# CrashCartCapital/rust-local-rag

Hardware: AMD Instinct MI355X
Metric: queries/sec, 768-d cosine top-100 over 10M chunks (single query, f32) (higher is better)
Workload: dtype f32

## Files before the change

rust-local-rag_amd/csrc/q8.hip:

```cpp
#include "common.h"
#include "kernels.h"
#include "../../include/rlr_gpu.h"

#include <algorithm>
#include <cstdlib>

namespace rlr {

namespace {

typedef unsigned int u32x4 __attribute__((ext_vector_type(4)));

__device__ inline float wave_max_abs(float v)
{
#pragma unroll
    for (int off = 32; off > 0; off >>= 1)
        v = fmaxf(v, __shfl_xor(v, off));
    return v;
}

__device__ inline float wave_add_all(float v)
{
#pragma unroll
    for (int off = 32; off > 0; off >>= 1)
        v += __shfl_xor(v, off);
    return v;
}

template <bool F16>
__global__ __launch_bounds__(256) void q8_build_kernel(const void *__restrict__ rows, uint32_t pitch_bytes, uint32_t dim,
                                                       uint32_t row_begin, uint32_t n_rows, uint8_t *__restrict__ q8,
                                                       float *__restrict__ scale, uint32_t *__restrict__ stats)
{
    const int lane = threadIdx.x & 63;
    const uint32_t row = row_begin + blockIdx.x * 4 + (threadIdx.x >> 6);
    if (row >= n_rows)
        return;
    const unsigned char *rowp = static_cast<const unsigned char *>(rows) + static_cast<size_t>(row) * pitch_bytes;
    auto elem = [&](uint32_t e) -> float {
        if constexpr (F16)
            return h2f(reinterpret_cast<const uint16_t *>(rowp)[e]);
        else
            return reinterpret_cast<const float *>(rowp)[e];
    };
    float m = 0.0f;
    bool has_nan = false, has_inf = false;
    for (uint32_t e = lane; e < dim; e += 64) {
        const float v = elem(e);
        has_nan |= v != v;
        has_inf |= __builtin_fabsf(v) > 3.4028234e38f;
        m = fmaxf(m, __builtin_fabsf(v));
    }
    has_nan = __ballot(has_nan) != 0;
    has_inf = __ballot(has_inf) != 0;
    const bool bad = has_nan || has_inf;
    m = wave_max_abs(m);
    const float s = (bad || m == 0.0f) ? 1.0f : m / 127.0f;
    float err2 = 0.0f;
    uint8_t *out = q8 + static_cast<size_t>(row) * dim;
    for (uint32_t e = lane; e < dim; e += 64) {
        const float v = bad ? 0.0f : elem(e);
        float k = __builtin_rintf(v / s);
        k = fminf(fmaxf(k, -127.0f), 127.0f);
        const float d = v - s * k;
        err2 += d * d;
        out[e] = static_cast<uint8_t>(static_cast<int>(k) + 128);
    }
    err2 = wave_add_all(err2);
    if (lane == 0) {
        scale[row] = bad ? __builtin_bit_cast(float, 0x7FC00000u) : s;
        if (has_inf && !has_nan)
            atomicOr(&stats[2], 1u);
        const float delta = __builtin_sqrtf(err2) * 1.001f + 1e-30f;
        if (!bad) {
            atomicMax(&stats[0], __builtin_bit_cast(uint32_t, delta));
            atomicMax(&stats[1], __builtin_bit_cast(uint32_t, s));
        }
    }
}

template <int B>
__device__ inline float ubyte_f32(uint32_t w)
{
    return static_cast<float>((w >> (8 * B)) & 0xFFu);
}

__device__ inline float dot16_u8(u32x4 x, const float (&q)[16], float acc)
{
    acc = __builtin_fmaf(ubyte_f32<0>(x[0]), q[0], acc);
    acc = __builtin_fmaf(ubyte_f32<1>(x[0]), q[1], acc);
    acc = __builtin_fmaf(ubyte_f32<2>(x[0]), q[2], acc);
    acc = __builtin_fmaf(ubyte_f32<3>(x[0]), q[3], acc);
    acc = __builtin_fmaf(ubyte_f32<0>(x[1]), q[4], acc);
    acc = __builtin_fmaf(ubyte_f32<1>(x[1]), q[5], acc);
    acc = __builtin_fmaf(ubyte_f32<2>(x[1]), q[6], acc);
    acc = __builtin_fmaf(ubyte_f32<3>(x[1]), q[7], acc);
    acc = __builtin_fmaf(ubyte_f32<0>(x[2]), q[8], acc);
    acc = __builtin_fmaf(ubyte_f32<1>(x[2]), q[9], acc);
    acc = __builtin_fmaf(ubyte_f32<2>(x[2]), q[10], acc);
    acc = __builtin_fmaf(ubyte_f32<3>(x[2]), q[11], acc);
    acc = __builtin_fmaf(ubyte_f32<0>(x[3]), q[12], acc);
    acc = __builtin_fmaf(ubyte_f32<1>(x[3]), q[13], acc);
    acc = __builtin_fmaf(ubyte_f32<2>(x[3]), q[14], acc);
    acc = __builtin_fmaf(ubyte_f32<3>(x[3]), q[15], acc);
    return acc;
}

template <int R, int L>
__global__ __launch_bounds__(256) void q8_scan_kernel(const uint8_t *__restrict__ q8, const float *__restrict__ scale,
                                                      const float *__restrict__ query, float *__restrict__ scores,
                                                      uint32_t *__restrict__ g_hist, uint32_t n_rows, uint32_t dim,
                                                      uint32_t group_rows)
{
    __shared__ uint32_t s_hist[kHistBins];
    const int tid = threadIdx.x;
    const int lane = tid & 63;
    const int wave = __builtin_amdgcn_readfirstlane(tid >> 6);
    for (int i = tid; i < kHistBins; i += 256)
        s_hist[i] = 0;
    const uint32_t p16 = dim / 16;
    bool active[L];
    float qv[L][16];
    float qs = 0.0f;
#pragma unroll
    for (int l = 0; l < L; ++l) {
        active[l] = static_cast<uint32_t>(lane + 64 * l) < p16;
#pragma unroll
        for (int b = 0; b < 16; ++b) {
            qv[l][b] = active[l] ? query[(lane + 64 * l) * 16 + b] : 0.0f;
            qs += qv[l][b];
        }
    }
    const float bias = 128.0f * qs;
    __syncthreads();

    const uint32_t n_groups = (n_rows + group_rows - 1) / group_rows;
    const uint32_t n_waves = gridDim.x * 4;
    for (uint32_t g = blockIdx.x * 4 + wave; g < n_groups; g += n_waves) {
        const uint32_t row0 = g * group_rows;
        const uint32_t nr = min(group_rows, n_rows - row0);
        float mine = 0.0f;
        for (uint32_t r = 0; r < nr; r += R) {
            u32x4 x[R][L];
            float sc[R];
#pragma unroll
            for (int rr = 0; rr < R; ++rr) {
                const uint32_t row = min(row0 + r + rr, row0 + nr - 1);
                const u32x4 *p = reinterpret_cast<const u32x4 *>(q8 + static_cast<size_t>(row) * dim) + lane;
#pragma unroll
                for (int l = 0; l < L; ++l)
                    x[rr][l] = active[l] ? __builtin_nontemporal_load(p + 64 * l)
                                         : u32x4{0x80808080u, 0x80808080u, 0x80808080u, 0x80808080u};
                sc[rr] = scale[row];
            }
#pragma unroll
            for (int rr = 0; rr < R; ++rr) {
                float acc = -bias;
#pragma unroll
                for (int l = 0; l < L; ++l)
                    acc = dot16_u8(x[rr][l], qv[l], acc);
                const float tot = wave_sum(acc);
                const float v = sc[rr] * tot;
                if (static_cast<uint32_t>(lane) == r + rr)
                    mine = v;
            }
        }
        if (static_cast<uint32_t>(lane) < nr) {
            scores[row0 + lane] = mine;
            if (g_hist)
                atomicAdd(&s_hist[score_key(mine) >> 21], 1u);
        }
    }
    if (g_hist) {
        __syncthreads();
        for (int i = tid; i < kHistBins; i += 256) {
            const uint32_t c = s_hist[i];
            if (c)
                atomicAdd(&g_hist[i], c);
        }
    }
}

template <int G, int NL, int NB>
__global__ __launch_bounds__(256) void q8_scan_packed_kernel(const uint8_t *__restrict__ q8, const float *__restrict__ scale,
                                                             const float *__restrict__ query, float *__restrict__ scores,
                                                             uint32_t *__restrict__ g_hist, uint32_t n_rows, uint32_t dim,
                                                             uint32_t group_rows)
{
    constexpr int RI = G * NB;
    static_assert(RI <= 64, "a group parks one score per lane");
    __shared__ uint32_t s_hist[kHistBins];
    const int tid = threadIdx.x;
    const int lane = tid & 63;
    const int wave = __builtin_amdgcn_readfirstlane(tid >> 6);
    for (int i = tid; i < kHistBins; i += 256)
        s_hist[i] = 0;
    const uint32_t p16 = dim / 16;
    uint32_t rib[NL], off[NL];
    float qv[NL][16], nbias[NL];
#pragma unroll
    for (int j = 0; j < NL; ++j) {
        const uint32_t u = static_cast<uint32_t>(j * 64 + lane);
        rib[j] = u / p16;
        const uint32_t seg = u - rib[j] * p16;
        off[j] = seg * 16;
        float qs = 0.0f;
#pragma unroll
        for (int b = 0; b < 16; ++b) {
            qv[j][b] = query[seg * 16 + b];
            qs += qv[j][b];
        }
        nbias[j] = -128.0f * qs;
    }
    __syncthreads();

    const uint32_t n_groups = (n_rows + group_rows - 1) / group_rows;
    const uint32_t n_waves = gridDim.x * 4;
    for (uint32_t g = blockIdx.x * 4 + wave; g < n_groups; g += n_waves) {
        const uint32_t row0 = g * group_rows;
        const uint32_t nr = min(group_rows, n_rows - row0);
        const uint32_t last = row0 + nr - 1;
        const float my_scale = scale[min(row0 + static_cast<uint32_t>(lane), last)];
        float mine = 0.0f;
        for (uint32_t r = 0; r < nr; r += RI) {
            u32x4 x[NB][NL];
#pragma unroll
            for (int bb = 0; bb < NB; ++bb)
#pragma unroll
                for (int j = 0; j < NL; ++j) {
                    const uint32_t row = min(row0 + r + bb * G + rib[j], last);
                    x[bb][j] = __builtin_nontemporal_load(reinterpret_cast<const u32x4 *>(q8 + static_cast<size_t>(row) * dim + off[j]));
                }
#pragma unroll
            for (int bb = 0; bb < NB; ++bb) {
                float acc[NL];
#pragma unroll
                for (int j = 0; j < NL; ++j)
                    acc[j] = dot16_u8(x[bb][j], qv[j], nbias[j]);
#pragma unroll
                for (int rb = 0; rb < G; ++rb) {
                    float part = 0.0f;
#pragma unroll
                    for (int j = 0; j < NL; ++j)
                        part += rib[j] == static_cast<uint32_t>(rb) ? acc[j] : 0.0f;
                    const float tot = wave_sum(part);
                    if (static_cast<uint32_t>(lane) == r + bb * G + rb)
                        mine = tot;
                }
            }
        }
        if (static_cast<uint32_t>(lane) < nr) {
            const float v = my_scale * mine;
            scores[row0 + lane] = v;
            if (g_hist)
                atomicAdd(&s_hist[score_key(v) >> 21], 1u);
        }
    }
    if (g_hist) {
        __syncthreads();
        for (int i = tid; i < kHistBins; i += 256) {
            const uint32_t c = s_hist[i];
            if (c)
                atomicAdd(&g_hist[i], c);
        }
    }
}

}

hipError_t launch_q8_build(const void *rows, uint32_t pitch16, uint32_t dim, int dtype, uint32_t row_begin, uint32_t n_rows,
                           void *q8, float *scale, uint32_t *stats, hipStream_t s)
{
    if (row_begin >= n_rows)
        return hipSuccess;
    const uint32_t blocks = (n_rows - row_begin + 3) / 4;
    if (dtype == RLR_F16)
        hipLaunchKernelGGL(q8_build_kernel<true>, dim3(blocks), dim3(256), 0, s, rows, pitch16 * 16, dim, row_begin, n_rows,
                           static_cast<uint8_t *>(q8), scale, stats);
    else
        hipLaunchKernelGGL(q8_build_kernel<false>, dim3(blocks), dim3(256), 0, s, rows, pitch16 * 16, dim, row_begin, n_rows,
                           static_cast<uint8_t *>(q8), scale, stats);
    return hipGetLastError();
}

hipError_t launch_q8_scan(const void *q8, const float *scale, uint32_t n_rows, uint32_t dim, const float *query,
                          float *scores, uint32_t *hist, int n_cu, hipStream_t s)
{
    if (n_rows == 0)
        return hipSuccess;
    static const int tune = [] {
        const char *v = getenv("RLR_Q8_VARIANT");
        return v ? static_cast<int>(strtol(v, nullptr, 0)) : 0;
    }();
    const int r = (tune & 0xFF) ? (tune & 0xFF) : 8;
    const uint32_t bpc = ((tune >> 8) & 0xFF) ? ((tune >> 8) & 0xFF) : 8;
    uint32_t group = ((tune >> 16) & 0xFF) ? ((tune >> 16) & 0xFF) : 32;
    group = std::max<uint32_t>(static_cast<uint32_t>(r), group / r * r);
    const uint32_t n_groups = (n_rows + group - 1) / group;
    const uint32_t blocks = std::max<uint32_t>(1, std::min<uint32_t>((n_groups + 3) / 4, static_cast<uint32_t>(n_cu) * bpc));
    const uint8_t *p = static_cast<const uint8_t *>(q8);
    static const bool packed = [] {
        const char *v = getenv("RLR_Q8_PACKED");
        return !(v && v[0] == '0');
    }();
    if (packed) {
        const uint32_t p16 = dim / 16;
#define RLR_Q8_PACKED_CASE(G_, NL_, NB_, GROUP_, BPC_)                                                                \
    if (p16 * G_ == NL_ * 64) {                                                                                      \
        const uint32_t pg = GROUP_;                                                                                  \
        const uint32_t pgroups = (n_rows + pg - 1) / pg;                                                             \
        const uint32_t pbpc = ((tune >> 8) & 0xFF) ? ((tune >> 8) & 0xFF) : BPC_;                                    \
        const uint32_t pblocks = std::max<uint32_t>(1, std::min<uint32_t>((pgroups + 3) / 4, static_cast<uint32_t>(n_cu) * pbpc)); \
        hipLaunchKernelGGL((q8_scan_packed_kernel<G_, NL_, NB_>), dim3(pblocks), dim3(256), 0, s, p, scale, query, scores, \
                           hist, n_rows, dim, pg);                                                                   \
        return hipGetLastError();                                                                                    \
    }
        RLR_Q8_PACKED_CASE(4, 3, 2, 32, 2)
        RLR_Q8_PACKED_CASE(8, 3, 1, 32, 4)
        RLR_Q8_PACKED_CASE(2, 3, 4, 32, 4)
        RLR_Q8_PACKED_CASE(2, 1, 8, 32, 8)
        RLR_Q8_PACKED_CASE(4, 1, 8, 32, 8)
        RLR_Q8_PACKED_CASE(8, 1, 8, 64, 8)
#undef RLR_Q8_PACKED_CASE
    }
    if (dim > 1024) {
        hipLaunchKernelGGL((q8_scan_kernel<4, 2>), dim3(blocks), dim3(256), 0, s, p, scale, query, scores, hist, n_rows, dim, group);
        return hipGetLastError();
    }
    switch (r) {
    case 4: hipLaunchKernelGGL((q8_scan_kernel<4, 1>), dim3(blocks), dim3(256), 0, s, p, scale, query, scores, hist, n_rows, dim, group); break;
    case 16: hipLaunchKernelGGL((q8_scan_kernel<16, 1>), dim3(blocks), dim3(256), 0, s, p, scale, query, scores, hist, n_rows, dim, group); break;
    default: hipLaunchKernelGGL((q8_scan_kernel<8, 1>), dim3(blocks), dim3(256), 0, s, p, scale, query, scores, hist, n_rows, dim, group); break;
    }
    return hipGetLastError();
}

float q8_arith_eps(uint32_t dim, float scale_max, float q_norm)
{
    return 32.0f * 5.9604645e-8f * 256.0f * __builtin_sqrtf(static_cast<float>(dim)) * q_norm * scale_max * 1.0625f;
}

}
```

Before: 224.5.

## Score int8 chunks with sdot4 against a three-plane integer query

Quantises the query into a 24-bit fixed-point integer split into three signed int8 planes. Each u8 chunk row is then scored with sdot4 integer dot products instead of per-byte float conversion plus FMA, and the three partial sums are recombined in double. Cross-lane reductions become integer DPP/shuffle fold trees that sum several rows at once rather than doing a full wave reduction per row. The default packed config for dim 768 changes to 4 rows per batch with one block per CU. This trades float ALU work for int dot instructions but adds query preprocessing, a fallback path for non-finite queries, and a small change in rounding behaviour.

```diff
diff --git a/rust-local-rag_amd/csrc/q8.hip b/rust-local-rag_amd/csrc/q8.hip
--- a/rust-local-rag_amd/csrc/q8.hip
+++ b/rust-local-rag_amd/csrc/q8.hip
@@ -79,6 +79,103 @@
     }
 }
 
+
+constexpr int kQ8Unit = 127 * 65793;
+
+__device__ inline bool q8_query_max(const float *__restrict__ query, uint32_t dim, int lane, float *qmax)
+{
+    float m = 0.0f;
+    bool bad = false;
+    for (uint32_t e = lane; e < dim; e += 64) {
+        const float a = __builtin_fabsf(query[e]);
+        bad |= !(a <= 3.4028234e38f);
+        m = fmaxf(m, a);
+    }
+    m = wave_max_abs(m);
+    *qmax = m;
+    return __ballot(bad) == 0 && m != 0.0f;
+}
+
+__device__ inline void q8_planes(const float *__restrict__ q16, bool active, double inv, u32x4 (&pl)[3])
+{
+#pragma unroll
+    for (int p = 0; p < 3; ++p)
+        pl[p] = u32x4{0u, 0u, 0u, 0u};
+#pragma unroll
+    for (int b = 0; b < 16; ++b) {
+        const double v = active ? static_cast<double>(q16[b]) : 0.0;
+        const int q = static_cast<int>(__builtin_rint(v * inv));
+        const int d0 = static_cast<int>(static_cast<int8_t>(q & 0xFF));
+        const int q1 = (q - d0) >> 8;
+        const int d1 = static_cast<int>(static_cast<int8_t>(q1 & 0xFF));
+        const int d2 = (q1 - d1) >> 8;
+        const int sh = 8 * (b & 3);
+        pl[0][b >> 2] |= static_cast<uint32_t>(d0 & 0xFF) << sh;
+        pl[1][b >> 2] |= static_cast<uint32_t>(d1 & 0xFF) << sh;
+        pl[2][b >> 2] |= static_cast<uint32_t>(d2 & 0xFF) << sh;
+    }
+}
+
+__device__ inline void dot16_i8(u32x4 x, const u32x4 (&pl)[3], int (&a)[3])
+{
+#pragma unroll
+    for (int w = 0; w < 4; ++w) {
+        const int s = static_cast<int>(x[w] ^ 0x80808080u);
+#pragma unroll
+        for (int p = 0; p < 3; ++p)
+            a[p] = __builtin_amdgcn_sdot4(s, static_cast<int>(pl[p][w]), a[p], false);
+    }
+}
+
+__device__ inline float q8_finish(const int (&a)[3], double unit, float scale)
+{
+    const double t = static_cast<double>(a[0]) + 256.0 * static_cast<double>(a[1]) + 65536.0 * static_cast<double>(a[2]);
+    return scale * static_cast<float>(t * unit);
+}
+
+template <int CTRL>
+__device__ inline int dpp_iadd(int v)
+{
+    return v + __builtin_amdgcn_update_dpp(0, v, CTRL, 0xF, 0xF, true);
+}
+
+template <int W>
+__device__ inline int run_sum(int v)
+{
+    if constexpr (W >= 2)
+        v = dpp_iadd<0xB1>(v);
+    if constexpr (W >= 4)
+        v = dpp_iadd<0x4E>(v);
+    if constexpr (W >= 8)
+        v = dpp_iadd<0x141>(v);
+    if constexpr (W >= 16)
+        v = dpp_iadd<0x140>(v);
+    if constexpr (W >= 32)
+        v += __shfl_xor(v, 16);
+    if constexpr (W >= 64)
+        v += __shfl_xor(v, 32);
+    return v;
+}
+
+template <int OFF>
+__device__ inline int fold_pair(int lo, int hi, bool up)
+{
+    const int keep = up ? hi : lo;
+    const int send = up ? lo : hi;
+    return keep + __shfl_xor(send, OFF);
+}
+
+__device__ inline void q8_hist_flush(const uint32_t *s_hist, uint32_t *__restrict__ g_hist, int tid)
+{
+    __syncthreads();
+    for (int i = tid; i < kHistBins; i += 256) {
+        const uint32_t c = s_hist[i];
+        if (c)
+            atomicAdd(&g_hist[i], c);
+    }
+}
+
+
 template <int B>
 __device__ inline float ubyte_f32(uint32_t w)
 {
@@ -107,17 +204,10 @@
 }
 
 template <int R, int L>
-__global__ __launch_bounds__(256) void q8_scan_kernel(const uint8_t *__restrict__ q8, const float *__restrict__ scale,
-                                                      const float *__restrict__ query, float *__restrict__ scores,
-                                                      uint32_t *__restrict__ g_hist, uint32_t n_rows, uint32_t dim,
-                                                      uint32_t group_rows)
-{
-    __shared__ uint32_t s_hist[kHistBins];
-    const int tid = threadIdx.x;
-    const int lane = tid & 63;
-    const int wave = __builtin_amdgcn_readfirstlane(tid >> 6);
-    for (int i = tid; i < kHistBins; i += 256)
-        s_hist[i] = 0;
+__device__ inline void q8_scan_float_body(const uint8_t *__restrict__ q8, const float *__restrict__ scale,
+                                          const float *__restrict__ query, float *__restrict__ scores, uint32_t *s_hist,
+                                          bool hist, uint32_t n_rows, uint32_t dim, uint32_t group_rows, int lane, int wave)
+{
     const uint32_t p16 = dim / 16;
     bool active[L];
     float qv[L][16];
@@ -132,7 +222,6 @@
         }
     }
     const float bias = 128.0f * qs;
-    __syncthreads();
 
     const uint32_t n_groups = (n_rows + group_rows - 1) / group_rows;
     const uint32_t n_waves = gridDim.x * 4;
@@ -167,34 +256,19 @@
         }
         if (static_cast<uint32_t>(lane) < nr) {
             scores[row0 + lane] = mine;
-            if (g_hist)
+            if (hist)
                 atomicAdd(&s_hist[score_key(mine) >> 21], 1u);
         }
     }
-    if (g_hist) {
-        __syncthreads();
-        for (int i = tid; i < kHistBins; i += 256) {
-            const uint32_t c = s_hist[i];
-            if (c)
-                atomicAdd(&g_hist[i], c);
-        }
-    }
 }
 
 template <int G, int NL, int NB>
-__global__ __launch_bounds__(256) void q8_scan_packed_kernel(const uint8_t *__restrict__ q8, const float *__restrict__ scale,
-                                                             const float *__restrict__ query, float *__restrict__ scores,
-                                                             uint32_t *__restrict__ g_hist, uint32_t n_rows, uint32_t dim,
-                                                             uint32_t group_rows)
+__device__ inline void q8_scan_packed_float_body(const uint8_t *__restrict__ q8, const float *__restrict__ scale,
+                                                 const float *__restrict__ query, float *__restrict__ scores,
+                                                 uint32_t *s_hist, bool hist, uint32_t n_rows, uint32_t dim,
+                                                 uint32_t group_rows, int lane, int wave)
 {
     constexpr int RI = G * NB;
-    static_assert(RI <= 64, "a group parks one score per lane");
-    __shared__ uint32_t s_hist[kHistBins];
-    const int tid = threadIdx.x;
-    const int lane = tid & 63;
-    const int wave = __builtin_amdgcn_readfirstlane(tid >> 6);
-    for (int i = tid; i < kHistBins; i += 256)
-        s_hist[i] = 0;
     const uint32_t p16 = dim / 16;
     uint32_t rib[NL], off[NL];
     float qv[NL][16], nbias[NL];
@@ -212,7 +286,6 @@
         }
         nbias[j] = -128.0f * qs;
     }
-    __syncthreads();
 
     const uint32_t n_groups = (n_rows + group_rows - 1) / group_rows;
     const uint32_t n_waves = gridDim.x * 4;
@@ -252,18 +325,212 @@
         if (static_cast<uint32_t>(lane) < nr) {
             const float v = my_scale * mine;
             scores[row0 + lane] = v;
+            if (hist)
+                atomicAdd(&s_hist[score_key(v) >> 21], 1u);
+        }
+    }
+}
+
+
+template <int R, int L>
+__global__ __launch_bounds__(256) void q8_scan_kernel(const uint8_t *__restrict__ q8, const float *__restrict__ scale,
+                                                      const float *__restrict__ query, float *__restrict__ scores,
+                                                      uint32_t *__restrict__ g_hist, uint32_t n_rows, uint32_t dim,
+                                                      uint32_t group_rows)
+{
+    static_assert(R == 4 || R == 8 || R == 16, "R rows fold into one vector in log2 R steps");
+    constexpr int W = 64 / R;
+    __shared__ uint32_t s_hist[kHistBins];
+    const int tid = threadIdx.x;
+    const int lane = tid & 63;
+    const int wave = __builtin_amdgcn_readfirstlane(tid >> 6);
+    for (int i = tid; i < kHistBins; i += 256)
+        s_hist[i] = 0;
+    __syncthreads();
+    float qmax;
+    if (!q8_query_max(query, dim, lane, &qmax)) {
+        q8_scan_float_body<R, L>(q8, scale, query, scores, s_hist, g_hist != nullptr, n_rows, dim, group_rows, lane, wave);
+        if (g_hist)
+            q8_hist_flush(s_hist, g_hist, tid);
+        return;
+    }
+    const double unit = static_cast<double>(qmax) / kQ8Unit;
+    const double inv = kQ8Unit / static_cast<double>(qmax);
+    const uint32_t p16 = dim / 16;
+    bool active[L];
+    u32x4 qp[L][3];
+#pragma unroll
+    for (int l = 0; l < L; ++l) {
+        active[l] = static_cast<uint32_t>(lane + 64 * l) < p16;
+        q8_planes(query + (active[l] ? (lane + 64 * l) * 16 : 0), active[l], inv, qp[l]);
+    }
+    uint32_t row_of = 0;
+#pragma unroll
+    for (int t = 0; (1 << t) < R; ++t)
+        row_of |= ((static_cast<uint32_t>(lane) >> (5 - t)) & 1u) << t;
+    const uint32_t slot = static_cast<uint32_t>(lane) & (W - 1);
+    const uint32_t my_row = slot * R + row_of;
+
+    const uint32_t n_groups = (n_rows + group_rows - 1) / group_rows;
+    const uint32_t n_waves = gridDim.x * 4;
+    for (uint32_t g = blockIdx.x * 4 + wave; g < n_groups; g += n_waves) {
+        const uint32_t row0 = g * group_rows;
+        const uint32_t nr = min(group_rows, n_rows - row0);
+        const uint32_t last = row0 + nr - 1;
+        const float my_scale = scale[min(row0 + my_row, last)];
+        int mine[3] = {0, 0, 0};
+        for (uint32_t r = 0; r < nr; r += R) {
+            u32x4 x[R][L];
+#pragma unroll
+            for (int rr = 0; rr < R; ++rr) {
+                const uint32_t row = min(row0 + r + rr, last);
+                const u32x4 *p = reinterpret_cast<const u32x4 *>(q8 + static_cast<size_t>(row) * dim) + lane;
+#pragma unroll
+                for (int l = 0; l < L; ++l)
+                    x[rr][l] = active[l] ? __builtin_nontemporal_load(p + 64 * l)
+                                         : u32x4{0x80808080u, 0x80808080u, 0x80808080u, 0x80808080u};
+            }
+            int a[R][3];
+#pragma unroll
+            for (int rr = 0; rr < R; ++rr) {
+                a[rr][0] = a[rr][1] = a[rr][2] = 0;
+#pragma unroll
+                for (int l = 0; l < L; ++l)
+                    dot16_i8(x[rr][l], qp[l], a[rr]);
+            }
+            const bool park = slot == r / R;
+#pragma unroll
+            for (int p = 0; p < 3; ++p) {
+                int v[R];
+#pragma unroll
+                for (int rr = 0; rr < R; ++rr)
+                    v[rr] = a[rr][p];
+#pragma unroll
+                for (int i = 0; i < R / 2; ++i)
+                    v[i] = fold_pair<32>(v[2 * i], v[2 * i + 1], (lane & 32) != 0);
+#pragma unroll
+                for (int i = 0; i < R / 4; ++i)
+                    v[i] = fold_pair<16>(v[2 * i], v[2 * i + 1], (lane & 16) != 0);
+                if constexpr (R >= 8) {
+#pragma unroll
+                    for (int i = 0; i < R / 8; ++i)
+                        v[i] = fold_pair<8>(v[2 * i], v[2 * i + 1], (lane & 8) != 0);
+                }
+                if constexpr (R >= 16)
+                    v[0] = fold_pair<4>(v[0], v[1], (lane & 4) != 0);
+                const int tot = run_sum<W>(v[0]);
+                mine[p] = park ? tot : mine[p];
+            }
+        }
+        if (my_row < nr) {
+            const float v = q8_finish(mine, unit, my_scale);
+            scores[row0 + my_row] = v;
             if (g_hist)
                 atomicAdd(&s_hist[score_key(v) >> 21], 1u);
         }
     }
-    if (g_hist) {
-        __syncthreads();
-        for (int i = tid; i < kHistBins; i += 256) {
-            const uint32_t c = s_hist[i];
-            if (c)
-                atomicAdd(&g_hist[i], c);
-        }
-    }
+    if (g_hist)
+        q8_hist_flush(s_hist, g_hist, tid);
+}
+
+template <int G, int NL, int NB>
+__global__ __launch_bounds__(256) void q8_scan_packed_kernel(const uint8_t *__restrict__ q8, const float *__restrict__ scale,
+                                                             const float *__restrict__ query, float *__restrict__ scores,
+                                                             uint32_t *__restrict__ g_hist, uint32_t n_rows, uint32_t dim,
+                                                             uint32_t group_rows)
+{
+    static_assert(NL == 1 || NL == 3, "whole rows per load, or rows cut 2 : 1");
+    constexpr int RI = G * NB;
+    constexpr int S = 64 / G;
+    constexpr int NP = NL == 1 ? 1 : 2;
+    static_assert(RI <= 64, "a group parks one score per lane");
+    __shared__ uint32_t s_hist[kHistBins];
+    const int tid = threadIdx.x;
+    const int lane = tid & 63;
+    const int wave = __builtin_amdgcn_readfirstlane(tid >> 6);
+    for (int i = tid; i < kHistBins; i += 256)
+        s_hist[i] = 0;
+    __syncthreads();
+    float qmax;
+    if (!q8_query_max(query, dim, lane, &qmax)) {
+        q8_scan_packed_float_body<G, NL, NB>(q8, scale, query, scores, s_hist, g_hist != nullptr, n_rows, dim, group_rows,
+                                             lane, wave);
+        if (g_hist)
+            q8_hist_flush(s_hist, g_hist, tid);
+        return;
+    }
+    const double unit = static_cast<double>(qmax) / kQ8Unit;
+    const double inv = kQ8Unit / static_cast<double>(qmax);
+    const uint32_t run = static_cast<uint32_t>(lane) / S, slot = static_cast<uint32_t>(lane) % S;
+    const uint32_t row_of = NL == 1 ? run : (run >> 1) + (run & 1u) * (G / 2);
+    uint32_t rib[NL], off[NL];
+    u32x4 qp[NP][3];
+    if constexpr (NL == 1) {
+        rib[0] = run;
+        off[0] = slot * 16;
+        q8_planes(query + slot * 16, true, inv, qp[0]);
+    } else {
+        const uint32_t long_unit = static_cast<uint32_t>(lane) % (2 * S);
+        rib[0] = static_cast<uint32_t>(lane) / (2 * S);
+        rib[1] = rib[0] + G / 2;
+        rib[2] = row_of;
+        off[0] = off[1] = long_unit * 16;
+        off[2] = (2 * S + slot) * 16;
+        q8_planes(query + long_unit * 16, true, inv, qp[0]);
+        q8_planes(query + (2 * S + slot) * 16, true, inv, qp[1]);
+    }
+    const uint32_t my_row = slot * G + row_of;
+
+    const uint32_t n_groups = (n_rows + group_rows - 1) / group_rows;
+    const uint32_t n_waves = gridDim.x * 4;
+    for (uint32_t g = blockIdx.x * 4 + wave; g < n_groups; g += n_waves) {
+        const uint32_t row0 = g * group_rows;
+        const uint32_t nr = min(group_rows, n_rows - row0);
+        const uint32_t last = row0 + nr - 1;
+        const float my_scale = scale[min(row0 + my_row, last)];
+        int mine[3] = {0, 0, 0};
+        for (uint32_t r = 0; r < nr; r += RI) {
+            u32x4 x[NB][NL];
+#pragma unroll
+            for (int bb = 0; bb < NB; ++bb)
+#pragma unroll
+                for (int j = 0; j < NL; ++j) {
+                    const uint32_t row = min(row0 + r + bb * G + rib[j], last);
+                    x[bb][j] = __builtin_nontemporal_load(reinterpret_cast<const u32x4 *>(q8 + static_cast<size_t>(row) * dim + off[j]));
+                }
+#pragma unroll
+            for (int bb = 0; bb < NB; ++bb) {
+                const bool park = slot == r / G + bb;
+                if constexpr (NL == 1) {
+                    int a[3] = {0, 0, 0};
+                    dot16_i8(x[bb][0], qp[0], a);
+#pragma unroll
+                    for (int p = 0; p < 3; ++p) {
+                        const int tot = run_sum<S>(a[p]);
+                        mine[p] = park ? tot : mine[p];
+                    }
+                } else {
+                    int a0[3] = {0, 0, 0}, a1[3] = {0, 0, 0}, a2[3] = {0, 0, 0};
+                    dot16_i8(x[bb][0], qp[0], a0);
+                    dot16_i8(x[bb][1], qp[0], a1);
+                    dot16_i8(x[bb][2], qp[1], a2);
+#pragma unroll
+                    for (int p = 0; p < 3; ++p) {
+                        const int tot = run_sum<S>(fold_pair<S>(a0[p], a1[p], (lane & S) != 0) + a2[p]);
+                        mine[p] = park ? tot : mine[p];
+                    }
+                }
+            }
+        }
+        if (my_row < nr) {
+            const float v = q8_finish(mine, unit, my_scale);
+            scores[row0 + my_row] = v;
+            if (g_hist)
+                atomicAdd(&s_hist[score_key(v) >> 21], 1u);
+        }
+    }
+    if (g_hist)
+        q8_hist_flush(s_hist, g_hist, tid);
 }
 
 }
@@ -295,9 +562,6 @@
     const int r = (tune & 0xFF) ? (tune & 0xFF) : 8;
     const uint32_t bpc = ((tune >> 8) & 0xFF) ? ((tune >> 8) & 0xFF) : 8;
     uint32_t group = ((tune >> 16) & 0xFF) ? ((tune >> 16) & 0xFF) : 32;
-    group = std::max<uint32_t>(static_cast<uint32_t>(r), group / r * r);
-    const uint32_t n_groups = (n_rows + group - 1) / group;
-    const uint32_t blocks = std::max<uint32_t>(1, std::min<uint32_t>((n_groups + 3) / 4, static_cast<uint32_t>(n_cu) * bpc));
     const uint8_t *p = static_cast<const uint8_t *>(q8);
     static const bool packed = [] {
         const char *v = getenv("RLR_Q8_PACKED");
@@ -307,7 +571,8 @@
         const uint32_t p16 = dim / 16;
 #define RLR_Q8_PACKED_CASE(G_, NL_, NB_, GROUP_, BPC_)                                                                \
     if (p16 * G_ == NL_ * 64) {                                                                                      \
-        const uint32_t pg = GROUP_;                                                                                  \
+        const uint32_t tg = (tune >> 16) & 0xFF;                                                                     \
+        const uint32_t pg = (tg && tg % (G_ * NB_) == 0 && tg <= 64 && tg / G_ <= 64 / G_) ? tg : GROUP_;            \
         const uint32_t pgroups = (n_rows + pg - 1) / pg;                                                             \
         const uint32_t pbpc = ((tune >> 8) & 0xFF) ? ((tune >> 8) & 0xFF) : BPC_;                                    \
         const uint32_t pblocks = std::max<uint32_t>(1, std::min<uint32_t>((pgroups + 3) / 4, static_cast<uint32_t>(n_cu) * pbpc)); \
@@ -315,7 +580,11 @@
                            hist, n_rows, dim, pg);                                                                   \
         return hipGetLastError();                                                                                    \
     }
-        RLR_Q8_PACKED_CASE(4, 3, 2, 32, 2)
+        if ((tune & 0xFF) == 4)
+            RLR_Q8_PACKED_CASE(4, 3, 1, 32, 1)
+        if ((tune & 0xFF) == 8)
+            RLR_Q8_PACKED_CASE(4, 3, 2, 32, 1)
+        RLR_Q8_PACKED_CASE(4, 3, 4, 32, 1)
         RLR_Q8_PACKED_CASE(8, 3, 1, 32, 4)
         RLR_Q8_PACKED_CASE(2, 3, 4, 32, 4)
         RLR_Q8_PACKED_CASE(2, 1, 8, 32, 8)
@@ -323,11 +592,15 @@
         RLR_Q8_PACKED_CASE(8, 1, 8, 64, 8)
 #undef RLR_Q8_PACKED_CASE
     }
+    const uint32_t rr = dim > 1024 ? 4u : (r == 4 || r == 16) ? static_cast<uint32_t>(r) : 8u;
+    group = std::min<uint32_t>(64, std::max<uint32_t>(rr, group / rr * rr));
+    const uint32_t n_groups = (n_rows + group - 1) / group;
+    const uint32_t blocks = std::max<uint32_t>(1, std::min<uint32_t>((n_groups + 3) / 4, static_cast<uint32_t>(n_cu) * bpc));
     if (dim > 1024) {
         hipLaunchKernelGGL((q8_scan_kernel<4, 2>), dim3(blocks), dim3(256), 0, s, p, scale, query, scores, hist, n_rows, dim, group);
         return hipGetLastError();
     }
-    switch (r) {
+    switch (rr) {
     case 4: hipLaunchKernelGGL((q8_scan_kernel<4, 1>), dim3(blocks), dim3(256), 0, s, p, scale, query, scores, hist, n_rows, dim, group); break;
     case 16: hipLaunchKernelGGL((q8_scan_kernel<16, 1>), dim3(blocks), dim3(256), 0, s, p, scale, query, scores, hist, n_rows, dim, group); break;
     default: hipLaunchKernelGGL((q8_scan_kernel<8, 1>), dim3(blocks), dim3(256), 0, s, p, scale, query, scores, hist, n_rows, dim, group); break;
```

Result: no change. 223.6 (-0.4%).
